# rostin79s/TFHE-AES

Measured on AMD Instinct MI355X. Metric: AES-128 CTR blocks/sec (FHE), higher is better.
Workload: dtype u64+f64; 1 GPU; configs[2]: 128 CTR blocks per GPU, Server::aes_encrypt 10 rounds (1280 bit-CBS/block), counters pre-incremented client-side; params=PARAM_OPT, blocks_per_gpu=128, total_blocks=128

## Files before the change

### tfhe_aes_amd/csrc/engine_launch.h

```cpp
#pragma once

#define MAX_CHUNK_BITS 32768ull
#define MAX_WOPBS_BITS 16u

namespace {

#define LATENCY_BATCH_BITS 256ull
#define K2_PAIR_MIN_BITS 768ull
struct K2Plan { int form; uint64_t units_main; uint32_t r_main; uint64_t units_tail; uint32_t r_tail; };
K2Plan k2_plan(uint64_t m, uint32_t cu_count, uint32_t k1, bool allow_pair = true)
{
    K2Plan pl{};
    if (m <= LATENCY_BATCH_BITS) { pl.form = 0; pl.units_main = m; pl.r_main = 1; return pl; }
    if (allow_pair && k1 == 5 && m > K2_PAIR_MIN_BITS) {
        pl.form = 2; pl.r_main = 6; pl.r_tail = 4;
        const uint64_t gens = (m + 6ull * cu_count - 1) / (6ull * cu_count);
        uint64_t nu = gens * cu_count;
        uint64_t four = 6 * nu >= m ? (6 * nu - m) / 2 : 0;
        if (four > nu) four = nu;
        if (four == nu && 4 * nu > m) { nu = (m + 3) / 4; four = nu; }
        pl.units_tail = four; pl.units_main = nu - four;
        return pl;
    }
    pl.form = 1;
    pl.r_main = k1 == 5 ? 3 : 8;
    pl.units_main = (m + pl.r_main - 1) / pl.r_main;
    if (k1 == 5) {
        const uint64_t slots = 2ull * cu_count;
        pl.r_tail = 2;
        if ((m + 1) / 2 <= cu_count) {
            pl.units_main = 0;
            pl.units_tail = (m + 1) / 2;
        } else if (pl.units_main > slots) {
            const uint64_t nu = slots * ((m + 3 * slots - 1) / (3 * slots));
            if (2 * nu <= m) {
                pl.units_tail = 3 * nu - m;
                pl.units_main = nu - pl.units_tail;
            }
        }
    }
    return pl;
}

#define AES_BLOCK_BITS 128ull
#define AES_WINDOW_MAX_BLOCKS (MAX_CHUNK_BITS / AES_BLOCK_BITS)
struct AesWindowPlan { uint64_t window, launches, generations, generations_by_round; };

uint64_t k2_generations(uint64_t m, uint32_t cu_count, uint32_t k1)
{
    if (m == 0) return 0;
    if (m <= K2_PAIR_MIN_BITS) return 1;
    const K2Plan pl = k2_plan(m, cu_count, k1);
    return (pl.units_main + pl.units_tail + cu_count - 1) / cu_count;
}

void aes_window_count(uint64_t n, uint64_t steps, uint64_t w, uint32_t cu_count, uint32_t k1, uint64_t *launches, uint64_t *generations)
{
    const uint64_t total = steps * n, full = total / w, rest = total % w;
    *launches = full + (rest ? 1 : 0);
    *generations = full * k2_generations(w * AES_BLOCK_BITS, cu_count, k1) + k2_generations(rest * AES_BLOCK_BITS, cu_count, k1);
}

AesWindowPlan aes_window_plan(uint64_t n, uint64_t steps, uint32_t cu_count, uint32_t k1, bool allow_pair = true)
{
    AesWindowPlan pl{};
    const uint64_t chunks = n / AES_WINDOW_MAX_BLOCKS, last = n % AES_WINDOW_MAX_BLOCKS;
    pl.launches = steps * (chunks + (last ? 1 : 0));
    pl.generations_by_round = steps * (chunks * k2_generations(MAX_CHUNK_BITS, cu_count, k1) + k2_generations(last * AES_BLOCK_BITS, cu_count, k1));
    pl.generations = pl.generations_by_round;
    if (n == 0 || steps == 0) return pl;
    const uint64_t gen_bits = 6ull * cu_count;
    if (k2_plan(std::min<uint64_t>(n * AES_BLOCK_BITS, MAX_CHUNK_BITS), cu_count, k1, allow_pair).form != 2) return pl;
    if (n * AES_BLOCK_BITS % gen_bits == 0) return pl;
    uint64_t g = AES_BLOCK_BITS, r = gen_bits;
    while (r) { const uint64_t t = g % r; g = r; r = t; }
    const uint64_t base = gen_bits / g;
    const uint64_t w = std::min<uint64_t>(n, AES_WINDOW_MAX_BLOCKS) / base * base;
    if (w == 0) return pl;
    uint64_t launches, generations;
    aes_window_count(n, steps, w, cu_count, k1, &launches, &generations);
    if (generations >= pl.generations_by_round) return pl;
    pl.window = w; pl.launches = launches; pl.generations = generations;
    return pl;
}

int launch_keyswitch(fheaes_ctx *c, const uint64_t *in, uint64_t m, uint64_t *out)
{
    if (m == 0) return FHEAES_OK;
    StageScope sc(c, FHEAES_STAGE_KEYSWITCH, m);
    const uint64_t ct_tiles16 = ((m + KS_CT_TILE - 1) / KS_CT_TILE) * (KS_CT_TILE / 16);
    TRY(ensure(c, c->ws_digits, ct_tiles16 * c->ks_ksteps * 1024));
    int8_t *af = (int8_t *)c->ws_digits.p;
    const uint64_t threads = ct_tiles16 * c->ks_ksteps * 64;
    ks_launch_digits_k1(dim3((unsigned)((threads + 255) / 256)), c->stream, in, (uint64_t)c->big1, c->big, m, c->ks_ksteps, af);
    KeyswitchArgs a{};
    a.afrag = af; a.bfrag = c->ksk_frag; a.ksteps = c->ks_ksteps; a.coltiles = c->ks_coltiles;
    a.in = in; a.in_stride = c->big1; a.body_index = (int32_t)c->big; a.body_col = c->n; a.ncols = c->n + 1;
    a.out = out; a.out_stride = c->n + 1; a.out_z_stride = 0; a.m = m;
    dim3 grid((c->ks_coltiles + KSL_COL_TILES - 1) / KSL_COL_TILES, (unsigned)((m + 16 * KSL_CT_TILES - 1) / (16 * KSL_CT_TILES)), 1);
    ks_launch_mfma_lds(1, grid, c->stream, a);
    HIP_TRY(c, hipGetLastError());
    return FHEAES_OK;
}

int launch_pfpks(fheaes_ctx *c, const uint64_t *in, uint64_t m, uint64_t *out, uint64_t out_stride, int block = -1)
{
    if (m == 0) return FHEAES_OK;
    StageScope sc(c, FHEAES_STAGE_PFPKS, m);
    const uint32_t gsz = c->k1 * FHE_N;
    const uint64_t ct_tiles16 = ((m + KS_CT_TILE - 1) / KS_CT_TILE) * (KS_CT_TILE / 16);
    TRY(ensure(c, c->ws_digits, ct_tiles16 * c->pf_ksteps * 2 * 1024));
    int8_t *af = (int8_t *)c->ws_digits.p;
    const uint64_t threads = ct_tiles16 * c->pf_ksteps * 64;
    ks_launch_digits_k3(dim3((unsigned)((threads + 255) / 256)), c->stream, in, (uint64_t)c->big1, c->big1, m, c->pf_ksteps, af);
    KeyswitchArgs a{};
    a.afrag = af; a.bfrag = c->pfpksk_frag; a.ksteps = c->pf_ksteps; a.coltiles = c->pf_coltiles;
    if (block >= 0) a.bfrag += (size_t)block * c->pf_ksteps * c->pf_coltiles * 8 * 1024;
    a.in = in; a.in_stride = c->big1; a.body_index = -1; a.body_col = 0; a.ncols = gsz;
    a.out = out; a.out_stride = out_stride; a.out_z_stride = block >= 0 ? 0 : gsz; a.m = m;
    dim3 grid((c->pf_coltiles + KSL_COL_TILES - 1) / KSL_COL_TILES, (unsigned)((m + 16 * KSL_CT_TILES - 1) / (16 * KSL_CT_TILES)), block >= 0 ? 1 : c->k1);
    ks_launch_mfma_lds(2, grid, c->stream, a);
    HIP_TRY(c, hipGetLastError());
    return FHEAES_OK;
}

int launch_forward_fourier(fheaes_ctx *c, const uint64_t *in, uint64_t polys, double2 *out, int stage)
{
    if (polys == 0) return FHEAES_OK;
    StageScope sc(c, stage, polys);
    uint64_t wgs = (polys + EP_GROUPS - 1) / EP_GROUPS;
    if (wgs > 8192) wgs = 8192;
    hipLaunchKernelGGL(forward_fourier_kernel, dim3((unsigned)wgs), dim3(EP_THREADS), 0, c->stream, in, out, polys, c->tw_d);
    HIP_TRY(c, hipGetLastError());
    return FHEAES_OK;
}

bool k2_pair_allowed(fheaes_ctx *c)
{
    if (c->k2_deny_pair) return false;
    if (c->k2_pair_ok < 0) {
        int per_cu = 0;
        const hipError_t oe = hipOccupancyMaxActiveBlocksPerMultiprocessor(&per_cu, blind_rotate_pair_kernel<5, 5, 8, 3, 2>, BRP_THREADS, 0);
        c->k2_pair_ok = (oe == hipSuccess && per_cu >= 1) ? 1 : 0;
        (void)hipGetLastError();
    }
    return c->k2_pair_ok == 1;
}

bool k2_home_allowed(fheaes_ctx *c)
{
    if (c->k1 != 5 || c->k2_deny_home) return false;
    if (c->k2_home < 0) {
        int per_cu = 0;
        const hipError_t oe = hipOccupancyMaxActiveBlocksPerMultiprocessor(&per_cu, blind_rotate16_kernel<5, 5, 8, 3, 2, true>, EP_THREADS, 0);
        c->k2_home = (oe == hipSuccess && per_cu >= 2) ? 1 : 0;
        (void)hipGetLastError();
    }
    return c->k2_home == 1;
}

static_assert(FHEAES_K2_PARK_SLOTS == BRP_PARK_SLOTS, "include/fheaes.h and kern_blindrot_pair.h disagree on the number of parking slots");
constexpr size_t PARK_OWNER_BYTES = BRP_PARK_SLOTS * sizeof(uint32_t) + BRP_PARK_TAIL_WORDS * sizeof(uint64_t);
constexpr size_t PARK_RECORD_PTR_OFFSET = BRP_PARK_SLOTS * sizeof(uint32_t) + 2 * sizeof(uint64_t);

int ensure_park_owner(fheaes_ctx *c)
{
    if (c->ws_park_owner.p) return FHEAES_OK;
    TRY(ensure(c, c->ws_park_owner, PARK_OWNER_BYTES));
    HIP_TRY(c, hipMemsetAsync(c->ws_park_owner.p, 0, PARK_OWNER_BYTES, c->stream));
    return FHEAES_OK;
}

size_t k2_pair_park_bytes(const fheaes_ctx *c, uint64_t grid)
{
    return (size_t)((c->k2_park_claim ? BRP_PARK_SLOTS : 0) + grid) * 2 * BRP_PARK_WORDS_PER_HALF * 8;
}

struct K2Launch {
    K2Plan pl;
    void (*kernel)(ExtProdArgs);
    const char *name;
    unsigned grid, threads;
    size_t park_bytes;
    bool park_owner;
};
K2Launch k2_launch(fheaes_ctx *c, uint64_t m)
{
    K2Launch L{};
    L.pl = k2_plan(m, c->cu_count, c->k1, k2_pair_allowed(c));
    L.grid = (unsigned)(L.pl.units_main + L.pl.units_tail);
    if (L.pl.form == 0) {
        L.threads = BL_THREADS;
        if (c->k1 == 5) { L.kernel = blind_rotate_latency_kernel<5, 5, 8>; L.name = "blind_rotate_latency_kernel<5,5,8>"; }
        else { L.kernel = blind_rotate_latency_kernel<2, 5, 8>; L.name = "blind_rotate_latency_kernel<2,5,8>"; }
    } else if (L.pl.form == 2) {
        L.threads = BRP_THREADS;
        L.kernel = blind_rotate_pair_kernel<5, 5, 8, 3, 2>;
        L.name = c->k2_park_claim ? "blind_rotate_pair_kernel<5,5,8,3,2> parking=claimed" : "blind_rotate_pair_kernel<5,5,8,3,2> parking=private";
        L.park_bytes = k2_pair_park_bytes(c, L.grid);
        L.park_owner = c->k2_park_claim != 0;
    } else {
        L.threads = EP_THREADS;
        if (c->k1 == 5 && k2_home_allowed(c)) { L.kernel = blind_rotate16_kernel<5, 5, 8, 3, 2, true>; L.name = "blind_rotate16_kernel<5,5,8,3,2,true>"; }
        else if (c->k1 == 5) { L.kernel = blind_rotate16_kernel<5, 5, 8, 3, 2, false>; L.name = "blind_rotate16_kernel<5,5,8,3,2,false>"; }
        else { L.kernel = blind_rotate16_kernel<2, 5, 8, 8>; L.name = "blind_rotate16_kernel<2,5,8,8,0,false>"; }
        L.park_bytes = (size_t)L.grid * BR16_PARK_WORDS_PER_WG * 8;
    }
    return L;
}

uint64_t aes_context_window(fheaes_ctx *c, uint64_t n, uint64_t steps)
{
    if (n == 0 || steps == 0 || c->aes_window == FHEAES_AES_WINDOW_OFF) return 0;
    if (c->aes_window) return std::min<uint64_t>(c->aes_window, std::min<uint64_t>(n, AES_WINDOW_MAX_BLOCKS));
    const bool pair = k2_launch(c, std::min<uint64_t>(n * AES_BLOCK_BITS, MAX_CHUNK_BITS)).pl.form == 2;
    return aes_window_plan(n, steps, c->cu_count, c->k1, pair).window;
}

int launch_cbs_pbs(fheaes_ctx *c, const uint64_t *lwe_small, uint64_t m, uint32_t level, uint64_t *out)
{
    if (m == 0) return FHEAES_OK;
    if ((uint64_t)c->n * c->p.pbs_level * c->k1 * c->k1 * FHE_H * 16 > 0x7FFFFFFFull)
        return c->fail(FHEAES_ERR_INVALID, "bootstrapping key larger than 2 GiB is not supported by the blind-rotation kernels");
    StageScope sc(c, FHEAES_STAGE_BLIND_ROTATE, m);
    ExtProdArgs a{};
    a.ggsw = c->bskf; a.tw = c->tw_d;
    a.out = out; a.count = m; a.iters = c->n; a.lwe_in = lwe_small;
    const uint64_t half_delta = 1ull << (64 - c->p.cbs_base_log * level - 1);
    a.tv_const = (uint64_t)0 - half_delta; a.body_shift = 1ull << 62; a.post_add = half_delta;
    const K2Launch L = k2_launch(c, m);
    if (L.pl.form != 0) a.units_main = (uint32_t)L.pl.units_main;
    if (L.park_bytes) {
        if (L.park_bytes > 0x7FFFFFFFull) return c->fail(FHEAES_ERR_INVALID, "internal: parking slab of %zu bytes exceeds one raw buffer", L.park_bytes);
        TRY(ensure(c, c->ws_park, L.park_bytes));
        a.park = (uint64_t *)c->ws_park.p; a.park_bytes = L.park_bytes;
    }
    if (L.park_owner) {
        TRY(ensure_park_owner(c));
        if (c->k2_park_pattern)
            HIP_TRY(c, hipMemcpyAsync(c->ws_park_owner.p, c->ws_park_pattern.p, BRP_PARK_SLOTS * sizeof(uint32_t), hipMemcpyDeviceToDevice, c->stream));
        else
            HIP_TRY(c, hipMemsetAsync(c->ws_park_owner.p, 0, BRP_PARK_SLOTS * sizeof(uint32_t), c->stream));
        a.park_owner = (uint32_t *)c->ws_park_owner.p;
        if (c->k2_park_record) {
            TRY(ensure(c, c->ws_park_record, (size_t)L.grid * 2 * sizeof(uint32_t)));
            HIP_TRY(c, hipMemsetAsync(c->ws_park_record.p, 0xFF, (size_t)L.grid * 2 * sizeof(uint32_t), c->stream));
            const uint64_t rp = (uint64_t)(uintptr_t)c->ws_park_record.p;
            uint32_t *const rp_word = (uint32_t *)((char *)c->ws_park_owner.p + PARK_RECORD_PTR_OFFSET);
            HIP_TRY(c, hipMemsetD32Async((hipDeviceptr_t)rp_word, (int)(uint32_t)rp, 1, c->stream));
            HIP_TRY(c, hipMemsetD32Async((hipDeviceptr_t)(rp_word + 1), (int)(uint32_t)(rp >> 32), 1, c->stream));
            c->k2_park_record_n = L.grid;
        }
    }
#ifdef EP_STAMPS
    static const char *namesL[EP_NPH] = {"barrier (result) + accumulate", "rotate+decompose (1 coeff x K1)", "read digits + forward fft", "digit stores", "barrier (digits)", "MAC", "barrier (MAC done)",
                                         "products store + next rows", "barrier (products)", "inverse fft -> doubles", "barrier (acc)", "barrier (decomposition)"};
    static const char *namesT[EP_NPH] = {"stage+rotate+decomp_first", "decomp_next", "fwd head", "pre-level barrier", "fwd tail (transpose+dft16)",
                                         "digit stores+late loads", "exchange barrier", "MAC", "products exchange", "inverse fft", "convert+add", "loop head"};
    StampReport rep(c, (size_t)L.grid * (L.threads / 64), L.pl.form == 0 ? namesL : namesT, L.pl.form == 0 ? 8 : 0);
    a.stamps = rep.d;
#endif
    hipLaunchKernelGGL(L.kernel, dim3(L.grid), dim3(L.threads), 0, c->stream, a);
    HIP_TRY(c, hipGetLastError());
    return FHEAES_OK;
}

int launch_vertical_packing(fheaes_ctx *c, const double2 *ggswf, uint64_t n_inputs, uint32_t bits, const uint64_t *luts,
                            uint32_t n_luts, int per_input, uint64_t *out)
{
    if (n_inputs == 0) return FHEAES_OK;
    StageScope sc(c, FHEAES_STAGE_VERTICAL_PACKING, n_inputs * n_luts * bits);
    const bool k4 = c->k1 == 5;
    const uint32_t R = k4 ? 3 : 8;
    void (*const cmux_kernel)(CmuxArgs) = k4 ? cmux_level_kernel<5, 15, 3> : cmux_level_kernel<2, 15, 8>;
    void (*const vp_kernel)(VpArgs) = k4 ? vertical_packing_kernel<5, 15, 3> : vertical_packing_kernel<2, 15, 8>;
    const uint32_t inst_per_input = n_luts * bits;
    const uint64_t W = lut_row_words(bits);
    const uint64_t *glwe_root = nullptr;
    if (bits > 9) {
        const uint32_t tree_bits = bits - 9;
        const uint64_t instances = n_inputs * inst_per_input, gsz = (uint64_t)c->k1 * FHE_N;
        const uint64_t half_words = instances * (1ull << (tree_bits - 1)) * gsz;
        TRY(ensure(c, c->ws_tree, 2 * half_words * 8));
        uint64_t *buf[2] = {(uint64_t *)c->ws_tree.p, (uint64_t *)c->ws_tree.p + half_words};
        for (uint32_t t = 0; t < tree_bits; ++t) {
            CmuxArgs a{};
            a.ggsw = ggswf; a.tw = c->tw_d;
            a.luts = t == 0 ? luts : nullptr; a.in = t == 0 ? nullptr : buf[(t - 1) & 1]; a.out = buf[t & 1];
            a.bits = bits; a.bit = 9 + t; a.nodes_out = 1u << (tree_bits - 1 - t);
            a.inst_per_input = inst_per_input; a.lut_per_input = per_input ? 1 : 0; a.lut_words = W;
            const uint64_t jobs = (uint64_t)inst_per_input * a.nodes_out;
            a.wg_per_input = (uint32_t)((jobs + R - 1) / R);
            hipLaunchKernelGGL(cmux_kernel, dim3((unsigned)(n_inputs * a.wg_per_input)), dim3(EP_THREADS), 0, c->stream, a);
            HIP_TRY(c, hipGetLastError());
        }
        glwe_root = buf[(tree_bits - 1) & 1];
    }
    VpArgs a{};
    a.ggsw = ggswf; a.tw = c->tw_d;
    a.out = out; a.iters = bits < 9 ? bits : 9; a.ggsw_per_input = bits;
    a.luts = luts; a.lut_words = W; a.glwe_in = glwe_root;
    a.lut_per_input = per_input ? 1 : 0; a.inst_per_input = inst_per_input;
    a.wg_per_input = (inst_per_input + R - 1) / R;
    hipLaunchKernelGGL(vp_kernel, dim3((unsigned)(n_inputs * a.wg_per_input)), dim3(EP_THREADS), 0, c->stream, a);
    HIP_TRY(c, hipGetLastError());
    return FHEAES_OK;
}

int noise_guard(fheaes_ctx *c, uint32_t level, const char *what)
{
    if (level > c->noise_level_seen) c->noise_level_seen = level;
    if (level > FHEAES_MAX_NOISE_LEVEL)
        return c->fail(FHEAES_ERR_INVALID, "%s would sum %u nominal-noise ciphertexts; the parameter set allows %u (MaxNoiseLevel, client.rs:92)", what, level,
                       (unsigned)FHEAES_MAX_NOISE_LEVEL);
    return FHEAES_OK;
}

struct KeySets {
    const uint64_t *rk;
    const uint32_t *of_block;
    uint64_t stride;
    uint32_t packed_glwes = 0, bit0 = 0;
    KeySets round(uint64_t r, uint64_t sw, uint64_t first_block = 0) const
    {
        const uint32_t *of = of_block ? of_block + first_block : nullptr;
        if (packed_glwes) return {rk, of, stride, packed_glwes, bit0 + (uint32_t)(r * AES_BLOCK_BITS)};
        return {rk + r * sw, of, stride};
    }
};

template <class F>
static void with_keys(const fheaes_ctx *c, const KeySets &k, F &&f)
{
    if (k.packed_glwes) f(PackedKeys{k.rk, k.stride, k.bit0, c->k});
    else f(LweKeys{k.rk, k.stride});
}

int launch_gather(fheaes_ctx *c, const uint64_t *src, uint32_t n_luts, const KeySets &k, uint64_t *out, uint64_t n_blocks, const GatherTable &t)
{
    if (n_blocks == 0) return FHEAES_OK;
    TRY(noise_guard(c, (uint32_t)t.terms + (k.rk ? 1u : 0u), "the linear layer (MixColumns / ShiftRows + AddRoundKey)"));
    StageScope sc(c, FHEAES_STAGE_LINEAR, n_blocks);
    dim3 grid((8 * c->big1 + 1023) / 1024, 16, (unsigned)n_blocks);
    with_keys(c, k, [&](auto keys) {
        hipLaunchKernelGGL(gather_add_kernel<decltype(keys)>, grid, dim3(256), 0, c->stream, src, n_luts, keys, k.of_block, out, n_blocks, c->big1, t);
    });
    HIP_TRY(c, hipGetLastError());
    return FHEAES_OK;
}

int launch_add_bcast(fheaes_ctx *c, uint64_t *dst, const KeySets &k, uint64_t words_per_block, uint64_t n_blocks)
{
    if (n_blocks == 0) return FHEAES_OK;
    TRY(noise_guard(c, 2, "the initial AddRoundKey"));
    StageScope sc(c, FHEAES_STAGE_LINEAR, n_blocks);
    const unsigned gx = (unsigned)std::min<uint64_t>((words_per_block + 255) / 256, 64);
    dim3 grid(gx, (unsigned)std::min<uint64_t>(n_blocks, std::max<uint64_t>(1, 16384 / gx)));
    with_keys(c, k, [&](auto keys) {
        hipLaunchKernelGGL(add_bcast_kernel<decltype(keys)>, grid, dim3(256), 0, c->stream, dst, keys, k.of_block, words_per_block, n_blocks, c->big1);
    });
    HIP_TRY(c, hipGetLastError());
    return FHEAES_OK;
}

int launch_key_rows(fheaes_ctx *c, uint64_t *dst, uint64_t dst_stride, const uint64_t *a, uint64_t a_stride, uint32_t rot, const uint64_t *b,
                    uint64_t b_stride, uint32_t rcon, uint32_t n_bytes, uint64_t n_keys, uint32_t level)
{
    if (level > 1) TRY(noise_guard(c, level, "a key-expansion word sum"));
    StageScope sc(c, FHEAES_STAGE_LINEAR, n_keys);
    dim3 grid((8 * c->big1 + 1023) / 1024, n_bytes, (unsigned)std::min<uint64_t>(n_keys, 65535));
    hipLaunchKernelGGL(key_rows_kernel, grid, dim3(256), 0, c->stream, dst, dst_stride, a, a_stride, rot, b, b_stride, rcon, c->big1, n_keys);
    HIP_TRY(c, hipGetLastError());
    return FHEAES_OK;
}

int launch_xts_tweaks(fheaes_ctx *c, const uint64_t *anchor, uint64_t anchor_stride, uint64_t n_units, uint32_t off0, uint32_t n_off, uint64_t *out)
{
    if (n_off == 0 || off0 > XTS_MAX_OFFSET || n_off > XTS_MAX_OFFSET + 1 - off0)
        return c->fail(FHEAES_ERR_INVALID, "XTS tweak offsets %u .. %u: one gather reaches offset %u at most", off0, off0 + n_off - 1, XTS_MAX_OFFSET);
    if (n_units == 0) return FHEAES_OK;
    uint32_t weight = 0, s[4];
    for (uint32_t j = off0; j < off0 + n_off; ++j)
        for (uint32_t i = 0; i < 128; ++i) weight = std::max(weight, xts_tweak_row(j, i, s));
    TRY(noise_guard(c, weight, "the XTS tweak layer (multiplication by alpha^j)"));
    StageScope sc(c, FHEAES_STAGE_LINEAR, n_units * n_off);
    const uint64_t rows = n_units * n_off * 128;
    hipLaunchKernelGGL(xts_tweak_kernel, dim3((unsigned)std::min<uint64_t>(rows, 1u << 20)), dim3(256), 0, c->stream, anchor, anchor_stride, out, n_units, off0,
                       n_off, c->big1);
    HIP_TRY(c, hipGetLastError());
    return FHEAES_OK;
}

int launch_xts_whiten(fheaes_ctx *c, uint64_t *dst, const uint64_t *src, const uint64_t *tweaks, const uint32_t *tweak_of_block, const uint8_t *clear,
                      uint64_t n_blocks, uint32_t level)
{
    if (n_blocks == 0) return FHEAES_OK;
    TRY(noise_guard(c, level, "the XTS whitening (tweak + block)"));
    StageScope sc(c, FHEAES_STAGE_LINEAR, n_blocks);
    const unsigned gx = (unsigned)std::min<uint64_t>((128ull * c->big1 + 255) / 256, 64);
    dim3 grid(gx, (unsigned)std::min<uint64_t>(n_blocks, std::max<uint64_t>(1, 16384 / gx)));
    hipLaunchKernelGGL(xts_whiten_kernel, grid, dim3(256), 0, c->stream, dst, src, tweaks, tweak_of_block, clear, n_blocks, c->big1);
    HIP_TRY(c, hipGetLastError());
    return FHEAES_OK;
}

int launch_mac_link(fheaes_ctx *c, uint64_t *dst, const uint64_t *a, const uint64_t *b, const MacSlot *slots, uint64_t n_slots, uint32_t level, const char *what)
{
    if (n_slots == 0) return FHEAES_OK;
    TRY(noise_guard(c, level, what));
    StageScope sc(c, FHEAES_STAGE_LINEAR, n_slots);
    const unsigned gx = (unsigned)std::min<uint64_t>((128ull * c->big1 + 255) / 256, 64);
    dim3 grid(gx, (unsigned)std::min<uint64_t>(n_slots, std::max<uint64_t>(1, 16384 / gx)));
    hipLaunchKernelGGL(mac_link_kernel, grid, dim3(256), 0, c->stream, dst, a, b, slots, n_slots, c->big1);
    HIP_TRY(c, hipGetLastError());
    return FHEAES_OK;
}

static_assert(PACK_N == FHE_N && PACK_N % PACK_FOLD_ROWS == 0, "kern_linear.h's packing kernels are written for N = 512");

static void launch_mod_switch(fheaes_ctx *c, const uint64_t *glwe, uint64_t n_glwe, uint32_t width, uint64_t *out)
{
    const uint32_t gsz = c->k1 * FHE_N;
    const uint64_t total = n_glwe * (gsz / 64 * width);
    hipLaunchKernelGGL(mod_switch_pack_kernel, dim3((unsigned)std::min<uint64_t>((total + 255) / 256, 65536)), dim3(256), 0, c->stream, glwe, n_glwe, gsz,
                       width, out);
}

int pack_dev(fheaes_ctx *c, const uint64_t *in, uint64_t m, uint64_t *out, uint32_t width = 64)
{
    if (m == 0) return FHEAES_OK;
    const uint64_t gsz = (uint64_t)c->k1 * FHE_N;
    uint64_t chunk = c->ws_ggsw.bytes / (gsz * 8) / FHE_N * FHE_N;
    if (chunk == 0) {
        chunk = std::min<uint64_t>((m + FHE_N - 1) / FHE_N * FHE_N, MAX_CHUNK_BITS);
        TRY(ensure(c, c->ws_ggsw, chunk * gsz * 8));
    }
    chunk = std::min<uint64_t>(chunk, MAX_CHUNK_BITS);
    if (width != 64) TRY(ensure(c, c->ws_tmp_a, (std::min<uint64_t>(chunk, m) + FHE_N - 1) / FHE_N * gsz * 8));
    uint64_t *ks = (uint64_t *)c->ws_ggsw.p;
    for (uint64_t t0 = 0; t0 < m; t0 += chunk) {
        const uint64_t mc = std::min<uint64_t>(chunk, m - t0), glwes = (mc + FHE_N - 1) / FHE_N;
        TRY(launch_pfpks(c, in + t0 * c->big1, mc, ks, gsz, (int)c->k));
        uint64_t *o = width == 64 ? out + t0 / FHE_N * gsz : (uint64_t *)c->ws_tmp_a.p;
        StageScope sc(c, FHEAES_STAGE_LINEAR, mc);
        HIP_TRY(c, hipMemsetAsync(o, 0, glwes * gsz * 8, c->stream));
        hipLaunchKernelGGL(pack_fold_kernel, dim3(FHE_N / PACK_FOLD_ROWS, c->k1, (unsigned)glwes), dim3(256), 0, c->stream, ks, mc, c->k1, o);
        HIP_TRY(c, hipGetLastError());
        if (width != 64) {
            launch_mod_switch(c, o, glwes, width, out + t0 / FHE_N * (gsz / 64 * width));
            HIP_TRY(c, hipGetLastError());
        }
    }
    return FHEAES_OK;
}

int unpack_dev(fheaes_ctx *c, const uint64_t *in, uint64_t m, uint64_t *out)
{
    for (uint64_t t0 = 0; t0 < m; t0 += MAX_CHUNK_BITS) {
        const uint64_t mc = std::min<uint64_t>(MAX_CHUNK_BITS, m - t0);
        StageScope sc(c, FHEAES_STAGE_LINEAR, mc);
        hipLaunchKernelGGL(sample_extract_kernel, dim3((unsigned)((mc + UNPACK_BITS_PER_WG - 1) / UNPACK_BITS_PER_WG)), dim3(256), 0, c->stream,
                           in + t0 / FHE_N * (uint64_t)c->k1 * FHE_N, mc, c->k, out + t0 * c->big1);
        HIP_TRY(c, hipGetLastError());
    }
    return FHEAES_OK;
}

int pack_keys_dev(fheaes_ctx *c, const uint64_t *in, uint64_t m, uint64_t n_keys, uint64_t *out)
{
    const uint64_t gsz = (uint64_t)c->k1 * FHE_N, glwes = (m + FHE_N - 1) / FHE_N, max_keys = MAX_CHUNK_BITS / m;
    uint64_t chunk = c->ws_ggsw.bytes / (gsz * 8) / m;
    if (chunk == 0) {
        chunk = std::min<uint64_t>(n_keys, max_keys);
        TRY(ensure(c, c->ws_ggsw, chunk * m * gsz * 8));
    }
    chunk = std::min<uint64_t>(chunk, max_keys);
    uint64_t *ks = (uint64_t *)c->ws_ggsw.p;
    for (uint64_t j0 = 0; j0 < n_keys; j0 += chunk) {
        const uint64_t kc = std::min<uint64_t>(chunk, n_keys - j0);
        TRY(launch_pfpks(c, in + j0 * m * c->big1, kc * m, ks, gsz, (int)c->k));
        uint64_t *o = out + j0 * glwes * gsz;
        StageScope sc(c, FHEAES_STAGE_LINEAR, kc * m);
        HIP_TRY(c, hipMemsetAsync(o, 0, kc * glwes * gsz * 8, c->stream));
        for (uint64_t j = 0; j < kc; ++j)
            hipLaunchKernelGGL(pack_fold_kernel, dim3(FHE_N / PACK_FOLD_ROWS, c->k1, (unsigned)glwes), dim3(256), 0, c->stream, ks + j * m * gsz, m, c->k1,
                               o + j * glwes * gsz);
        HIP_TRY(c, hipGetLastError());
    }
    return FHEAES_OK;
}

int unpack_keys_dev(fheaes_ctx *c, const uint64_t *in, uint64_t m, uint64_t n_keys, uint64_t *out)
{
    const uint64_t key_words = (m + FHE_N - 1) / FHE_N * c->k1 * FHE_N;
    for (uint64_t j = 0; j < n_keys; ++j) TRY(unpack_dev(c, in + j * key_words, m, out + j * m * c->big1));
    return FHEAES_OK;
}

int mod_switch_dev(fheaes_ctx *c, const uint64_t *in, uint64_t n_glwe, uint32_t width, uint64_t *out)
{
    const uint64_t gsz = (uint64_t)c->k1 * FHE_N, step = MAX_CHUNK_BITS / FHE_N;
    for (uint64_t g0 = 0; g0 < n_glwe; g0 += step) {
        const uint64_t gc = std::min<uint64_t>(step, n_glwe - g0);
        StageScope sc(c, FHEAES_STAGE_LINEAR, gc * FHE_N);
        launch_mod_switch(c, in + g0 * gsz, gc, width, out + g0 * (gsz / 64 * width));
        HIP_TRY(c, hipGetLastError());
    }
    return FHEAES_OK;
}

int unpack_mod_dev(fheaes_ctx *c, const uint64_t *in, uint64_t m, uint32_t width, uint64_t *out)
{
    for (uint64_t t0 = 0; t0 < m; t0 += MAX_CHUNK_BITS) {
        const uint64_t mc = std::min<uint64_t>(MAX_CHUNK_BITS, m - t0);
        StageScope sc(c, FHEAES_STAGE_LINEAR, mc);
        hipLaunchKernelGGL(sample_extract_mod_kernel, dim3((unsigned)((mc + UNPACK_BITS_PER_WG - 1) / UNPACK_BITS_PER_WG)), dim3(256), 0, c->stream,
                           in + t0 / FHE_N * (uint64_t)c->k1 * 8 * width, mc, c->k, width, out + t0 * c->big1);
        HIP_TRY(c, hipGetLastError());
    }
    return FHEAES_OK;
}

int expand_lwe_dev(fheaes_ctx *c, const MaskKey &key, uint64_t first_index, const uint64_t *bodies, uint64_t m, uint64_t *out)
{
    for (uint64_t t0 = 0; t0 < m; t0 += MAX_CHUNK_BITS) {
        const uint64_t mc = std::min<uint64_t>(MAX_CHUNK_BITS, m - t0);
        StageScope sc(c, FHEAES_STAGE_LINEAR, mc);
        hipLaunchKernelGGL(expand_lwe_kernel, dim3((unsigned)((mc * c->k + 3) / 4)), dim3(256), 0, c->stream, out + t0 * c->big1, bodies + t0, mc, c->k,
                           first_index + t0, key);
        HIP_TRY(c, hipGetLastError());
    }
    return FHEAES_OK;
}

int check_keys(fheaes_ctx *c)
{
    if (!c) return FHEAES_ERR_INVALID;
    if (!c->have_keys) return c->fail(FHEAES_ERR_NOKEYS, "evaluation keys have not been uploaded");
    return FHEAES_OK;
}

int ensure_wopbs_ws(fheaes_ctx *c, uint64_t bits)
{
    const uint64_t ggsw_words = (uint64_t)c->k1 * c->k1 * FHE_N;
    TRY(ensure(c, c->ws_small, bits * (c->n + 1) * 8));
    TRY(ensure(c, c->ws_pbs, bits * c->big1 * 8));
    TRY(ensure(c, c->ws_ggsw, bits * ggsw_words * 8));
    TRY(ensure(c, c->ws_ggswf, bits * ggsw_words * 8));
    return FHEAES_OK;
}

int wopbs_dev(fheaes_ctx *c, const uint64_t *lwe_in, uint64_t n_inputs, uint32_t bits, const uint64_t *luts, uint32_t n_luts,
              int per_input, uint64_t *lwe_out)
{
    if (bits < 1 || bits > MAX_WOPBS_BITS) return c->fail(FHEAES_ERR_INVALID, "bits_per_input must be in 1..%u (got %u)", MAX_WOPBS_BITS, bits);
    if (n_luts < 1) return c->fail(FHEAES_ERR_INVALID, "n_luts must be >= 1");
    if (n_inputs == 0) return FHEAES_OK;
    uint64_t chunk_inputs = std::max<uint64_t>(1, MAX_CHUNK_BITS / bits);
    if (bits > 9) {
        const uint64_t per_input = (uint64_t)n_luts * bits * (1ull << (bits - 9)) * c->k1 * FHE_N * 8;
        chunk_inputs = std::max<uint64_t>(1, std::min<uint64_t>(chunk_inputs, (2ull << 30) / per_input));
    }
    const uint64_t W = lut_row_words(bits);
    const uint64_t ggsw_words = (uint64_t)c->k1 * c->k1 * FHE_N;
    TRY(ensure_wopbs_ws(c, std::min<uint64_t>(n_inputs, chunk_inputs) * bits));
    for (uint64_t i0 = 0; i0 < n_inputs; i0 += chunk_inputs) {
        const uint64_t ni = std::min<uint64_t>(chunk_inputs, n_inputs - i0);
        const uint64_t m = ni * bits;
        const uint64_t *in = lwe_in + i0 * bits * c->big1;
        TRY(launch_keyswitch(c, in, m, (uint64_t *)c->ws_small.p));
        TRY(launch_cbs_pbs(c, (const uint64_t *)c->ws_small.p, m, 1, (uint64_t *)c->ws_pbs.p));
        TRY(launch_pfpks(c, (const uint64_t *)c->ws_pbs.p, m, (uint64_t *)c->ws_ggsw.p, ggsw_words));
        TRY(launch_forward_fourier(c, (const uint64_t *)c->ws_ggsw.p, m * c->k1 * c->k1, (double2 *)c->ws_ggswf.p, FHEAES_STAGE_GGSW_FFT));
        const uint64_t *l = per_input ? luts + i0 * n_luts * bits * W : luts;
        TRY(launch_vertical_packing(c, (const double2 *)c->ws_ggswf.p, ni, bits, l, n_luts, per_input, lwe_out + i0 * n_luts * bits * c->big1));
    }
    return FHEAES_OK;
}

}
```

### tfhe_aes_amd/csrc/kern_keyswitch.h

```cpp
#pragma once
#include <hip/hip_runtime.h>
#include <stdint.h>
#include "fft_dev.h"

#define KS_CT_TILE 64
#define KS_KSTEP 64

typedef int ks_int4 __attribute__((ext_vector_type(4)));

struct KeyswitchArgs {
    const int8_t *afrag;
    const int8_t *bfrag;
    uint32_t ksteps, coltiles;
    const uint64_t *in;
    uint64_t in_stride;
    int32_t body_index;
    uint32_t body_col;
    uint32_t ncols;
    uint64_t *out;
    uint64_t out_stride, out_z_stride;
    uint64_t m;
};

#define KSL_CT_TILES 8
#define KSL_THREADS (64 * KSL_CT_TILES)
#define KSL_COL_TILES 4

#ifndef FHEAES_KS_DECLS_ONLY
__global__ __launch_bounds__(256) void keybytes_kernel(const uint64_t *key, uint64_t key_z_stride, uint32_t rows, uint32_t ncols,
                                                       uint32_t ksteps, uint32_t coltiles, int8_t *frag)
{
    const uint64_t gid = (uint64_t)blockIdx.x * blockDim.x + threadIdx.x;
    const uint32_t lane = gid & 63;
    const uint64_t t = gid >> 6;
    const uint32_t C = t % coltiles;
    const uint32_t ks = (uint32_t)(t / coltiles);
    const uint32_t z = blockIdx.y;
    if (ks >= ksteps) return;
    const uint32_t col = C * 16 + (lane & 15);
    const uint32_t row0 = ks * KS_KSTEP + (lane >> 4) * 16;
    int8_t b[8][16];
#pragma unroll
    for (int e = 0; e < 16; ++e) {
        uint64_t x = 0;
        if (col < ncols && row0 + e < rows) x = key[(uint64_t)z * key_z_stride + (uint64_t)(row0 + e) * ncols + col];
        uint32_t carry = 0;
#pragma unroll
        for (int j = 0; j < 8; ++j) {
            uint32_t v = (uint32_t)((x >> (8 * j)) & 0xFF) + carry;
            carry = v >= 128 ? 1u : 0u;
            b[j][e] = (int8_t)(v & 0xFF);
        }
    }
    int8_t *o = frag + ((((uint64_t)z * ksteps + ks) * coltiles + C) * 8) * 1024 + (uint64_t)lane * 16;
#pragma unroll
    for (int j = 0; j < 8; ++j) {
        ks_int4 w;
        memcpy(&w, b[j], 16);
        *reinterpret_cast<ks_int4 *>(o + (uint64_t)j * 1024) = w;
    }
}

template <int BASE_LOG, int LEVELS, int PLANES>
__global__ __launch_bounds__(256) void digits_kernel(const uint64_t *in, uint64_t in_stride, uint32_t n_in, uint64_t m,
                                                     uint32_t ksteps, int8_t *frag)
{
    const uint64_t gid = (uint64_t)blockIdx.x * blockDim.x + threadIdx.x;
    const uint32_t lane = gid & 63;
    const uint64_t t = gid >> 6;
    const uint32_t ks = t % ksteps;
    const uint64_t T = t / ksteps;
    const uint64_t ct = T * 16 + (lane & 15);
    const uint32_t q0 = ks * KS_KSTEP + (lane >> 4) * 16;
    int8_t lo[16], hi[16];
#pragma unroll
    for (int e = 0; e < 16; ++e) { lo[e] = 0; hi[e] = 0; }
    if (ct < m) {
        const uint32_t i0 = q0 / LEVELS;
        constexpr int NI = (16 + LEVELS - 1) / LEVELS + 1;
#pragma unroll
        for (int ii = 0; ii < NI; ++ii) {
            const uint32_t i = i0 + ii;
            if (i >= n_in) break;
            int d[LEVELS];
            decompose_all<BASE_LOG, LEVELS>(in[ct * in_stride + i], d);
#pragma unroll
            for (int l = 0; l < LEVELS; ++l) {
                const int e = (int)(i * LEVELS + l) - (int)q0;
                if (e >= 0 && e < 16) {
                    const int dl = ((d[l] + 128) & 255) - 128;
#pragma unroll
                    for (int ee = 0; ee < 16; ++ee) if (ee == e) { lo[ee] = (int8_t)dl; hi[ee] = (int8_t)((d[l] - dl) >> 8); }
                }
            }
        }
    }
    int8_t *o = frag + ((T * ksteps + ks) * PLANES) * 1024 + (uint64_t)lane * 16;
    ks_int4 w;
    memcpy(&w, lo, 16);
    *reinterpret_cast<ks_int4 *>(o) = w;
    if (PLANES == 2) {
        memcpy(&w, hi, 16);
        *reinterpret_cast<ks_int4 *>(o + 1024) = w;
    }
}

template <int PLANES>
__global__ __launch_bounds__(KSL_THREADS, 2) void keyswitch_mfma_lds_kernel(const KeyswitchArgs A)
{
    constexpr int A_FRAGS = KSL_CT_TILES * PLANES;
    constexpr int B_FRAGS = KSL_COL_TILES * 8;
    constexpr int FRAGS = A_FRAGS + B_FRAGS;
    __shared__ __attribute__((aligned(16))) int8_t lds[2 * FRAGS * 1024];
    const int lane = threadIdx.x & 63, wave = threadIdx.x >> 6;
    const int wc = wave & 3, wt = wave >> 2;
    const uint32_t C0 = blockIdx.x * KSL_COL_TILES;
    const uint64_t T0 = (uint64_t)blockIdx.y * KSL_CT_TILES;
    const uint32_t z = blockIdx.z;
    const uint64_t ct_tiles_total = (A.m + 15) / 16;

    ks_int4 acc[4][8];
#pragma unroll
    for (int t = 0; t < 4; ++t)
#pragma unroll
        for (int s = 0; s < 8; ++s) acc[t][s] = (ks_int4){0, 0, 0, 0};

    auto issue = [&](uint32_t ks, int buf) {
        constexpr int WAVES = KSL_THREADS / 64;
#pragma unroll
        for (int i = 0; i < (FRAGS + WAVES - 1) / WAVES; ++i) {
            const int f = wave + WAVES * i;
            if (f < FRAGS) {
                const int8_t *src;
                if (f < A_FRAGS) {
                    uint64_t T = T0 + f / PLANES;
                    if (T >= ct_tiles_total) T = ct_tiles_total - 1;
                    src = A.afrag + ((T * A.ksteps + ks) * PLANES + (f % PLANES)) * 1024;
                } else {
                    const int g = f - A_FRAGS;
                    uint32_t C = C0 + g / 8;
                    if (C >= A.coltiles) C = A.coltiles - 1;
                    src = A.bfrag + ((((uint64_t)z * A.ksteps + ks) * A.coltiles + C) * 8 + (g % 8)) * 1024;
                }
                __builtin_amdgcn_global_load_lds((const __attribute__((address_space(1))) void *)(src + lane * 16),
                                                 (__attribute__((address_space(3))) void *)(lds + ((size_t)buf * FRAGS + f) * 1024), 16, 0, 0);
            }
        }
    };

    issue(0, 0);
    for (uint32_t ks = 0; ks < A.ksteps; ++ks) {
        const int buf = ks & 1;
        asm volatile("s_waitcnt vmcnt(0)" ::: "memory");
        __syncthreads();
        if (ks + 1 < A.ksteps) issue(ks + 1, buf ^ 1);
        const int8_t *base = lds + (size_t)buf * FRAGS * 1024 + lane * 16;
        ks_int4 a[4][PLANES], b[8];
#pragma unroll
        for (int s = 0; s < 8; ++s) b[s] = *reinterpret_cast<const ks_int4 *>(base + (A_FRAGS + wc * 8 + s) * 1024);
#pragma unroll
        for (int t = 0; t < 4; ++t)
#pragma unroll
            for (int pl = 0; pl < PLANES; ++pl) a[t][pl] = *reinterpret_cast<const ks_int4 *>(base + ((wt * 4 + t) * PLANES + pl) * 1024);
#pragma unroll
        for (int s = 0; s < 8; ++s) {
#pragma unroll
            for (int t = 0; t < 4; ++t) acc[t][s] = __builtin_amdgcn_mfma_i32_16x16x64_i8(a[t][0], b[s], acc[t][s], 0, 0, 0);
            if (PLANES == 2 && s >= 1) {
#pragma unroll
                for (int t = 0; t < 4; ++t) acc[t][s] = __builtin_amdgcn_mfma_i32_16x16x64_i8(a[t][1], b[s - 1], acc[t][s], 0, 0, 0);
            }
        }
    }

    const uint32_t C = C0 + wc;
    const uint32_t col = C * 16 + (lane & 15);
    if (C >= A.coltiles || col >= A.ncols) return;
#pragma unroll
    for (int t = 0; t < 4; ++t)
#pragma unroll
        for (int r = 0; r < 4; ++r) {
            const uint64_t ct = (T0 + wt * 4 + t) * 16 + (uint64_t)(lane >> 4) * 4 + r;
            if (ct >= A.m) continue;
            uint64_t v = 0;
#pragma unroll
            for (int s = 0; s < 8; ++s) v += (uint64_t)(int64_t)acc[t][s][r] << (8 * s);
            v = (uint64_t)0 - v;
            if (A.body_index >= 0 && col == A.body_col) v += A.in[ct * A.in_stride + (uint32_t)A.body_index];
            A.out[ct * A.out_stride + (uint64_t)z * A.out_z_stride + col] = v;
        }
}
#endif
```

### tfhe_aes_amd/csrc/ks_launch.h

```cpp
#pragma once
#ifdef FHEAES_SPLIT_KS
#ifndef FHEAES_KS_TU
#define FHEAES_KS_DECLS_ONLY
#endif
#endif
#include "kern_keyswitch.h"

#if defined(FHEAES_SPLIT_KS) && !defined(FHEAES_KS_TU)
#define FHEAES_KS_LAUNCH_DECL
#else
#define FHEAES_KS_LAUNCH_DEFINE
#ifdef FHEAES_SPLIT_KS
#define FHEAES_KS_LAUNCH_LINKAGE
#else
#define FHEAES_KS_LAUNCH_LINKAGE static inline
#endif
#endif

#ifdef FHEAES_KS_LAUNCH_DECL
void ks_launch_digits_k1(dim3 grid, hipStream_t s, const uint64_t *in, uint64_t in_stride, uint32_t n_in, uint64_t m, uint32_t ksteps, int8_t *frag);
void ks_launch_digits_k3(dim3 grid, hipStream_t s, const uint64_t *in, uint64_t in_stride, uint32_t n_in, uint64_t m, uint32_t ksteps, int8_t *frag);
void ks_launch_mfma_lds(int planes, dim3 grid, hipStream_t s, const KeyswitchArgs &a);
void ks_launch_keybytes(dim3 grid, hipStream_t s, const uint64_t *key, uint64_t key_z_stride, uint32_t rows, uint32_t ncols, uint32_t ksteps,
                        uint32_t coltiles, int8_t *frag);
#endif

#ifdef FHEAES_KS_LAUNCH_DEFINE
FHEAES_KS_LAUNCH_LINKAGE void ks_launch_digits_k1(dim3 grid, hipStream_t s, const uint64_t *in, uint64_t in_stride, uint32_t n_in, uint64_t m, uint32_t ksteps, int8_t *frag)
{
    hipLaunchKernelGGL((digits_kernel<2, 6, 1>), grid, dim3(256), 0, s, in, in_stride, n_in, m, ksteps, frag);
}
FHEAES_KS_LAUNCH_LINKAGE void ks_launch_digits_k3(dim3 grid, hipStream_t s, const uint64_t *in, uint64_t in_stride, uint32_t n_in, uint64_t m, uint32_t ksteps, int8_t *frag)
{
    hipLaunchKernelGGL((digits_kernel<12, 3, 2>), grid, dim3(256), 0, s, in, in_stride, n_in, m, ksteps, frag);
}
FHEAES_KS_LAUNCH_LINKAGE void ks_launch_mfma_lds(int planes, dim3 grid, hipStream_t s, const KeyswitchArgs &a)
{
    if (planes == 1) hipLaunchKernelGGL((keyswitch_mfma_lds_kernel<1>), grid, dim3(KSL_THREADS), 0, s, a);
    else hipLaunchKernelGGL((keyswitch_mfma_lds_kernel<2>), grid, dim3(KSL_THREADS), 0, s, a);
}
FHEAES_KS_LAUNCH_LINKAGE void ks_launch_keybytes(dim3 grid, hipStream_t s, const uint64_t *key, uint64_t key_z_stride, uint32_t rows, uint32_t ncols, uint32_t ksteps,
                                          uint32_t coltiles, int8_t *frag)
{
    hipLaunchKernelGGL(keybytes_kernel, grid, dim3(256), 0, s, key, key_z_stride, rows, ncols, ksteps, coltiles, frag);
}
#endif
```

Baseline: 58.49 blocks/s.

## Stage keyswitch inputs in LDS for digit packing and add dedicated k1 MFMA kernel

```diff
diff --git a/tfhe_aes_amd/csrc/engine_launch.h b/tfhe_aes_amd/csrc/engine_launch.h
--- a/tfhe_aes_amd/csrc/engine_launch.h
+++ b/tfhe_aes_amd/csrc/engine_launch.h
@@ -91,13 +91,12 @@
     const uint64_t ct_tiles16 = ((m + KS_CT_TILE - 1) / KS_CT_TILE) * (KS_CT_TILE / 16);
     TRY(ensure(c, c->ws_digits, ct_tiles16 * c->ks_ksteps * 1024));
     int8_t *af = (int8_t *)c->ws_digits.p;
-    const uint64_t threads = ct_tiles16 * c->ks_ksteps * 64;
-    ks_launch_digits_k1(dim3((unsigned)((threads + 255) / 256)), c->stream, in, (uint64_t)c->big1, c->big, m, c->ks_ksteps, af);
+    ks_launch_digits_k1(dim3(), c->stream, in, (uint64_t)c->big1, c->big, m, c->ks_ksteps, af);
     KeyswitchArgs a{};
     a.afrag = af; a.bfrag = c->ksk_frag; a.ksteps = c->ks_ksteps; a.coltiles = c->ks_coltiles;
     a.in = in; a.in_stride = c->big1; a.body_index = (int32_t)c->big; a.body_col = c->n; a.ncols = c->n + 1;
     a.out = out; a.out_stride = c->n + 1; a.out_z_stride = 0; a.m = m;
-    dim3 grid((c->ks_coltiles + KSL_COL_TILES - 1) / KSL_COL_TILES, (unsigned)((m + 16 * KSL_CT_TILES - 1) / (16 * KSL_CT_TILES)), 1);
+    dim3 grid((c->ks_coltiles + K1L_COL_TILES - 1) / K1L_COL_TILES, (unsigned)((m + 16 * K1L_CT_TILES - 1) / (16 * K1L_CT_TILES)), 1);
     ks_launch_mfma_lds(1, grid, c->stream, a);
     HIP_TRY(c, hipGetLastError());
     return FHEAES_OK;
@@ -111,8 +110,7 @@
     const uint64_t ct_tiles16 = ((m + KS_CT_TILE - 1) / KS_CT_TILE) * (KS_CT_TILE / 16);
     TRY(ensure(c, c->ws_digits, ct_tiles16 * c->pf_ksteps * 2 * 1024));
     int8_t *af = (int8_t *)c->ws_digits.p;
-    const uint64_t threads = ct_tiles16 * c->pf_ksteps * 64;
-    ks_launch_digits_k3(dim3((unsigned)((threads + 255) / 256)), c->stream, in, (uint64_t)c->big1, c->big1, m, c->pf_ksteps, af);
+    ks_launch_digits_k3(dim3(), c->stream, in, (uint64_t)c->big1, c->big1, m, c->pf_ksteps, af);
     KeyswitchArgs a{};
     a.afrag = af; a.bfrag = c->pfpksk_frag; a.ksteps = c->pf_ksteps; a.coltiles = c->pf_coltiles;
     if (block >= 0) a.bfrag += (size_t)block * c->pf_ksteps * c->pf_coltiles * 8 * 1024;
diff --git a/tfhe_aes_amd/csrc/kern_keyswitch.h b/tfhe_aes_amd/csrc/kern_keyswitch.h
--- a/tfhe_aes_amd/csrc/kern_keyswitch.h
+++ b/tfhe_aes_amd/csrc/kern_keyswitch.h
@@ -25,6 +25,9 @@
 #define KSL_CT_TILES 8
 #define KSL_THREADS (64 * KSL_CT_TILES)
 #define KSL_COL_TILES 4
+#define K1L_CT_TILES 16
+#define K1L_THREADS 256
+#define K1L_COL_TILES 2
 
 #ifndef FHEAES_KS_DECLS_ONLY
 __global__ __launch_bounds__(256) void keybytes_kernel(const uint64_t *key, uint64_t key_z_stride, uint32_t rows, uint32_t ncols,
@@ -61,47 +64,69 @@
     }
 }
 
+#define KSD_KSTEPS 8
+#define KSD_THREADS 256
+
 template <int BASE_LOG, int LEVELS, int PLANES>
-__global__ __launch_bounds__(256) void digits_kernel(const uint64_t *in, uint64_t in_stride, uint32_t n_in, uint64_t m,
-                                                     uint32_t ksteps, int8_t *frag)
+__global__ __launch_bounds__(KSD_THREADS) void digits_kernel(const uint64_t *in, uint64_t in_stride, uint32_t n_in, uint64_t m,
+                                                             uint32_t ksteps, int8_t *frag)
 {
-    const uint64_t gid = (uint64_t)blockIdx.x * blockDim.x + threadIdx.x;
-    const uint32_t lane = gid & 63;
-    const uint64_t t = gid >> 6;
-    const uint32_t ks = t % ksteps;
-    const uint64_t T = t / ksteps;
-    const uint64_t ct = T * 16 + (lane & 15);
-    const uint32_t q0 = ks * KS_KSTEP + (lane >> 4) * 16;
-    int8_t lo[16], hi[16];
-#pragma unroll
-    for (int e = 0; e < 16; ++e) { lo[e] = 0; hi[e] = 0; }
-    if (ct < m) {
+    constexpr int NI = (15 + LEVELS - 1) / LEVELS + 1;
+    constexpr int WORDS = (KSD_KSTEPS * KS_KSTEP - 16) / LEVELS + 1 + NI;
+    constexpr int STRIDE = WORDS | 1;
+    constexpr int WAVES = KSD_THREADS / 64;
+    static_assert(NI * LEVELS <= 24 && (LEVELS - 1) + 16 <= NI * LEVELS && LEVELS <= 8, "the byte string is six dwords, the shift below 64 bits");
+    __shared__ uint64_t words[16 * STRIDE];
+    const uint32_t lane = threadIdx.x & 63, wave = threadIdx.x >> 6;
+    const uint32_t runs = (ksteps + KSD_KSTEPS - 1) / KSD_KSTEPS;
+    const uint64_t T = blockIdx.x / runs;
+    const uint32_t ks0 = (blockIdx.x % runs) * KSD_KSTEPS;
+    const uint32_t i_lo = ks0 * KS_KSTEP / LEVELS;
+
+#pragma unroll
+    for (int cc = 0; cc < 16 / WAVES; ++cc) {
+        const uint32_t c = wave + WAVES * cc;
+        const uint64_t ct = T * 16 + c;
+        const uint64_t *row = in + ct * in_stride + i_lo;
+#pragma unroll
+        for (int jj = 0; jj < (WORDS + 63) / 64; ++jj) {
+            const uint32_t j = lane + 64 * jj;
+            if (j < WORDS) words[c * STRIDE + j] = (ct < m && i_lo + j < n_in) ? row[j] : 0;
+        }
+    }
+    __syncthreads();
+
+    const uint32_t c = lane & 15;
+#pragma unroll
+    for (int it = 0; it < KSD_KSTEPS / WAVES; ++it) {
+        const uint32_t ks = ks0 + it * WAVES + wave;
+        if (ks >= ksteps) break;
+        const uint32_t q0 = ks * KS_KSTEP + (lane >> 4) * 16;
         const uint32_t i0 = q0 / LEVELS;
-        constexpr int NI = (16 + LEVELS - 1) / LEVELS + 1;
+        const uint32_t shift = 8 * (q0 - i0 * LEVELS);
+        uint32_t lo[6] = {0, 0, 0, 0, 0, 0}, hi[6] = {0, 0, 0, 0, 0, 0};
 #pragma unroll
         for (int ii = 0; ii < NI; ++ii) {
-            const uint32_t i = i0 + ii;
-            if (i >= n_in) break;
             int d[LEVELS];
-            decompose_all<BASE_LOG, LEVELS>(in[ct * in_stride + i], d);
+            decompose_all<BASE_LOG, LEVELS>(words[c * STRIDE + (i0 - i_lo) + ii], d);
 #pragma unroll
             for (int l = 0; l < LEVELS; ++l) {
-                const int e = (int)(i * LEVELS + l) - (int)q0;
-                if (e >= 0 && e < 16) {
-                    const int dl = ((d[l] + 128) & 255) - 128;
-#pragma unroll
-                    for (int ee = 0; ee < 16; ++ee) if (ee == e) { lo[ee] = (int8_t)dl; hi[ee] = (int8_t)((d[l] - dl) >> 8); }
-                }
-            }
-        }
-    }
-    int8_t *o = frag + ((T * ksteps + ks) * PLANES) * 1024 + (uint64_t)lane * 16;
-    ks_int4 w;
-    memcpy(&w, lo, 16);
-    *reinterpret_cast<ks_int4 *>(o) = w;
-    if (PLANES == 2) {
-        memcpy(&w, hi, 16);
-        *reinterpret_cast<ks_int4 *>(o + 1024) = w;
+                const int b = ii * LEVELS + l;
+                const int dl = ((d[l] + 128) & 255) - 128;
+                lo[b >> 2] |= (uint32_t)(dl & 255) << (8 * (b & 3));
+                if (PLANES == 2) hi[b >> 2] |= (uint32_t)(((d[l] - dl) >> 8) & 255) << (8 * (b & 3));
+            }
+        }
+        int8_t *o = frag + ((T * ksteps + ks) * PLANES) * 1024 + (uint64_t)lane * 16;
+        ks_int4 w;
+#pragma unroll
+        for (int k = 0; k < 4; ++k) w[k] = (int)(uint32_t)((((uint64_t)lo[k + 1] << 32) | lo[k]) >> shift);
+        *reinterpret_cast<ks_int4 *>(o) = w;
+        if (PLANES == 2) {
+#pragma unroll
+            for (int k = 0; k < 4; ++k) w[k] = (int)(uint32_t)((((uint64_t)hi[k + 1] << 32) | hi[k]) >> shift);
+            *reinterpret_cast<ks_int4 *>(o + 1024) = w;
+        }
     }
 }
 
@@ -190,4 +215,94 @@
             A.out[ct * A.out_stride + (uint64_t)z * A.out_z_stride + col] = v;
         }
 }
+
+__global__ __launch_bounds__(K1L_THREADS) __attribute__((amdgpu_waves_per_eu(1, 1))) void keyswitch_mfma_k1_kernel(const KeyswitchArgs A)
+{
+    constexpr int A_FRAGS = K1L_CT_TILES;
+    constexpr int B_FRAGS = K1L_COL_TILES * 8;
+    constexpr int FRAGS = A_FRAGS + B_FRAGS;
+    constexpr int WAVES = K1L_THREADS / 64;
+    __shared__ __attribute__((aligned(16))) int8_t lds[2 * FRAGS * 1024];
+    const int lane = threadIdx.x & 63, wave = __builtin_amdgcn_readfirstlane(threadIdx.x >> 6);
+    const int wc = wave & 1, wt = wave >> 1;
+    const uint32_t C0 = blockIdx.x * K1L_COL_TILES;
+    const uint64_t T0 = (uint64_t)blockIdx.y * K1L_CT_TILES;
+    const uint64_t ct_tiles_total = (A.m + 15) / 16;
+    const uint32_t ksteps = A.ksteps;
+
+    ks_int4 acc[8][8];
+#pragma unroll
+    for (int t = 0; t < 8; ++t)
+#pragma unroll
+        for (int s = 0; s < 8; ++s) acc[t][s] = (ks_int4){0, 0, 0, 0};
+
+    auto issue = [&](uint32_t ks, int buf) {
+#pragma unroll
+        for (int i = 0; i < FRAGS / WAVES; ++i) {
+            const int f = wave + WAVES * i;
+            const int8_t *src;
+            if (f < A_FRAGS) {
+                uint64_t T = T0 + f;
+                if (T >= ct_tiles_total) T = ct_tiles_total - 1;
+                src = A.afrag + (T * ksteps + ks) * 1024;
+            } else {
+                const int g = f - A_FRAGS;
+                uint32_t C = C0 + g / 8;
+                if (C >= A.coltiles) C = A.coltiles - 1;
+                src = A.bfrag + (((uint64_t)ks * A.coltiles + C) * 8 + (g % 8)) * 1024;
+            }
+            __builtin_amdgcn_global_load_lds((const __attribute__((address_space(1))) void *)(src + lane * 16),
+                                             (__attribute__((address_space(3))) void *)(lds + ((size_t)buf * FRAGS + f) * 1024), 16, 0, 0);
+        }
+    };
+    auto landed = [&]() {
+        asm volatile("s_waitcnt vmcnt(0)" ::: "memory");
+        __syncthreads();
+    };
+    ks_int4 a[8], b[8];
+    issue(0, 0);
+    for (uint32_t ks = 0; ks < ksteps; ++ks) {
+        const int buf = ks & 1;
+        const int8_t *base = lds + (size_t)buf * FRAGS * 1024 + lane * 16;
+        auto key_plane = [&](int s) { b[s] = *reinterpret_cast<const ks_int4 *>(base + (A_FRAGS + wc * 8 + s) * 1024); };
+        landed();
+        key_plane(0);
+#pragma unroll
+        for (int t = 0; t < 8; ++t) a[t] = *reinterpret_cast<const ks_int4 *>(base + (wt * 8 + t) * 1024);
+        key_plane(1);
+        __builtin_amdgcn_sched_barrier(0);
+#pragma unroll
+        for (int s = 0; s < 8; ++s) {
+            if (s + 2 < 8) key_plane(s + 2);
+            if (s == 0 && ks + 1 < ksteps) issue(ks + 1, buf ^ 1);
+#pragma unroll
+            for (int t = 0; t < 8; ++t) acc[t][s] = __builtin_amdgcn_mfma_i32_16x16x64_i8(a[t], b[s], acc[t][s], 0, 0, 0);
+            __builtin_amdgcn_sched_barrier(0);
+        }
+    }
+
+    const uint32_t C = C0 + wc;
+    const uint32_t col = C * 16 + (lane & 15);
+    if (C >= A.coltiles || col >= A.ncols) return;
+    const bool body = A.body_index >= 0 && col == A.body_col;
+#pragma unroll
+    for (int t = 0; t < 8; ++t) {
+#pragma unroll
+        for (int u = t + 1; u < 8; ++u)
+            asm volatile("" : "+a"(acc[u][0]), "+a"(acc[u][1]), "+a"(acc[u][2]), "+a"(acc[u][3]), "+a"(acc[u][4]), "+a"(acc[u][5]), "+a"(acc[u][6]), "+a"(acc[u][7]));
+        const uint64_t ct0 = (T0 + wt * 8 + t) * 16 + (uint64_t)(lane >> 4) * 4;
+#pragma unroll
+        for (int r = 0; r < 4; ++r) {
+            const uint64_t ct = ct0 + r;
+            uint64_t v = 0;
+#pragma unroll
+            for (int s = 0; s < 8; ++s) v += (uint64_t)(int64_t)acc[t][s][r] << (8 * s);
+            v = (uint64_t)0 - v;
+            if (ct < A.m) {
+                if (body) v += A.in[ct * A.in_stride + (uint32_t)A.body_index];
+                A.out[ct * A.out_stride + col] = v;
+            }
+        }
+    }
+}
 #endif
diff --git a/tfhe_aes_amd/csrc/ks_launch.h b/tfhe_aes_amd/csrc/ks_launch.h
--- a/tfhe_aes_amd/csrc/ks_launch.h
+++ b/tfhe_aes_amd/csrc/ks_launch.h
@@ -26,17 +26,22 @@
 #endif
 
 #ifdef FHEAES_KS_LAUNCH_DEFINE
-FHEAES_KS_LAUNCH_LINKAGE void ks_launch_digits_k1(dim3 grid, hipStream_t s, const uint64_t *in, uint64_t in_stride, uint32_t n_in, uint64_t m, uint32_t ksteps, int8_t *frag)
+static inline dim3 ks_digits_grid(uint64_t m, uint32_t ksteps)
 {
-    hipLaunchKernelGGL((digits_kernel<2, 6, 1>), grid, dim3(256), 0, s, in, in_stride, n_in, m, ksteps, frag);
+    const uint64_t ct_tiles16 = ((m + KS_CT_TILE - 1) / KS_CT_TILE) * (KS_CT_TILE / 16);
+    return dim3((unsigned)(ct_tiles16 * ((ksteps + KSD_KSTEPS - 1) / KSD_KSTEPS)));
 }
-FHEAES_KS_LAUNCH_LINKAGE void ks_launch_digits_k3(dim3 grid, hipStream_t s, const uint64_t *in, uint64_t in_stride, uint32_t n_in, uint64_t m, uint32_t ksteps, int8_t *frag)
+FHEAES_KS_LAUNCH_LINKAGE void ks_launch_digits_k1(dim3, hipStream_t s, const uint64_t *in, uint64_t in_stride, uint32_t n_in, uint64_t m, uint32_t ksteps, int8_t *frag)
 {
-    hipLaunchKernelGGL((digits_kernel<12, 3, 2>), grid, dim3(256), 0, s, in, in_stride, n_in, m, ksteps, frag);
+    hipLaunchKernelGGL((digits_kernel<2, 6, 1>), ks_digits_grid(m, ksteps), dim3(KSD_THREADS), 0, s, in, in_stride, n_in, m, ksteps, frag);
+}
+FHEAES_KS_LAUNCH_LINKAGE void ks_launch_digits_k3(dim3, hipStream_t s, const uint64_t *in, uint64_t in_stride, uint32_t n_in, uint64_t m, uint32_t ksteps, int8_t *frag)
+{
+    hipLaunchKernelGGL((digits_kernel<12, 3, 2>), ks_digits_grid(m, ksteps), dim3(KSD_THREADS), 0, s, in, in_stride, n_in, m, ksteps, frag);
 }
 FHEAES_KS_LAUNCH_LINKAGE void ks_launch_mfma_lds(int planes, dim3 grid, hipStream_t s, const KeyswitchArgs &a)
 {
-    if (planes == 1) hipLaunchKernelGGL((keyswitch_mfma_lds_kernel<1>), grid, dim3(KSL_THREADS), 0, s, a);
+    if (planes == 1) hipLaunchKernelGGL(keyswitch_mfma_k1_kernel, grid, dim3(K1L_THREADS), 0, s, a);
     else hipLaunchKernelGGL((keyswitch_mfma_lds_kernel<2>), grid, dim3(KSL_THREADS), 0, s, a);
 }
 FHEAES_KS_LAUNCH_LINKAGE void ks_launch_keybytes(dim3 grid, hipStream_t s, const uint64_t *key, uint64_t key_z_stride, uint32_t rows, uint32_t ncols, uint32_t ksteps,
```

After: 58.78 blocks/s, median of 6. About the same (+0.5%).
